# 23skdu/longbow

Measured on AMD Instinct MI355X. Metric: k-NN queries/sec (batch=1024, k=100), 1Mx768 f32, higher is better.
Workload: dtype f32

## Files before the change

### longbow_amd/csrc/kernels_gemm.hip

```cpp
#include "lb_admit.h"

#include <cstdlib>

namespace lb {

constexpr int BM = 128;
constexpr int BN = 128;
constexpr int BK = 32;
constexpr int GEMM_THREADS = 256;

struct GemmArgs {
    const float *X;
    const float *norm2;
    const float *rnorm;
    int64_t row_begin, row_end;
    int D;
    const float *Q;
    int nq;
    const uint8_t *mask;
    const uint32_t *rowmap;
    CandState cs;
    int n_row_tiles, n_q_tiles;
    int boot;
};

__device__ __forceinline__ int swz_off(int row, int chunk)
{
    return row * BK + ((chunk ^ ((row >> 1) & 7)) << 2);
}

template <int MODE>
__device__ __forceinline__ f32x4 load_chunk(const float *base, int64_t row, int D, int k)
{
    f32x4 v = {0.f, 0.f, 0.f, 0.f};
    const float *p = base + row * (int64_t)D + k;
    if (MODE == 2) {
        v = *reinterpret_cast<const f32x4 *>(p);
    } else if (MODE == 1) {
        if (k < D) v = *reinterpret_cast<const f32x4 *>(p);
    } else {
        if (k + 0 < D) v.x = p[0];
        if (k + 1 < D) v.y = p[1];
        if (k + 2 < D) v.z = p[2];
        if (k + 3 < D) v.w = p[3];
    }
    return v;
}

template <int METRIC, int ALIGNED>
__global__ __launch_bounds__(GEMM_THREADS, 2) void gemm_filter_kernel(GemmArgs a)
{
    constexpr bool GLDS = ALIGNED == 2;
    const int b = blockIdx.x;
    const int xcd = b & 7;
    const int in_xcd = b >> 3;
    const int qt = in_xcd % a.n_q_tiles;
    const int rt = (in_xcd / a.n_q_tiles) * 8 + xcd;
    if (rt >= a.n_row_tiles) return;

    __shared__ __attribute__((aligned(16))) float lds_all[2 * 2 * BM * BK + BM + BM + BM / 4];
    float(*lds)[2][BM * BK] = reinterpret_cast<float(*)[2][BM * BK]>(lds_all);
    float *s_aux = lds_all + 2 * 2 * BM * BK;
    uint32_t *s_rowid = reinterpret_cast<uint32_t *>(s_aux + BM);
    uint8_t *s_vis = reinterpret_cast<uint8_t *>(s_rowid + BM);

    const int tid = threadIdx.x;
    const int lane = tid & 63;
    const int wave = tid >> 6;
    const int wr = wave >> 1, wc = wave & 1;
    const int l31 = lane & 31, h = lane >> 5;

    const int64_t row0 = a.row_begin + (int64_t)rt * BM;
    const int q0 = qt * BN;
    const int64_t last_row = a.row_end - 1;
    const int last_q = a.nq - 1;

    auto corpus_row = [&](int64_t pos) -> int64_t {
        if (pos > last_row) pos = last_row;
        return a.rowmap ? (int64_t)a.rowmap[pos] : pos;
    };
    const int64_t side_ri = corpus_row(row0 + (tid & (BM - 1)));

    int st_row[4], st_ch[4];
    int64_t st_xrow[4];
    int st_qrow[4];
#pragma unroll
    for (int i = 0; i < 4; i++) {
        int c = tid + GEMM_THREADS * i;
        st_row[i] = c >> 3;
        st_ch[i] = c & 7;
        st_xrow[i] = corpus_row(row0 + st_row[i]);
        int qr = q0 + st_row[i];
        st_qrow[i] = qr < last_q ? qr : last_q;
    }

    f32x16 acc[2][2];
#pragma unroll
    for (int i = 0; i < 2; i++)
#pragma unroll
        for (int j = 0; j < 2; j++)
#pragma unroll
            for (int r = 0; r < 16; r++) acc[i][j][r] = 0.f;

    const int nk = (a.D + BK - 1) / BK;
    f32x4 ra[4], rb[4];

    const float *gsrcA[4], *gsrcB[4];
    if (GLDS) {
#pragma unroll
        for (int i = 0; i < 4; i++) {
            const int j = wave * 4 + i;
            const int row = j * 8 + (lane >> 3);
            const int c = (lane & 7) ^ ((row >> 1) & 7);
            const int64_t xr = corpus_row(row0 + row);
            int qr = q0 + row;
            if (qr > last_q) qr = last_q;
            gsrcA[i] = a.X + xr * (int64_t)a.D + 4 * c;
            gsrcB[i] = a.Q + (int64_t)qr * a.D + 4 * c;
        }
    }
    const int wave_u = __builtin_amdgcn_readfirstlane(wave);
    auto glds_piece = [&](int p, int stage, int k0) {
        const int i = p >> 1;
        const int j = wave_u * 4 + i;
        if ((p & 1) == 0)
            __builtin_amdgcn_global_load_lds(
                (const __attribute__((address_space(1))) void *)(gsrcA[i] + k0),
                (__attribute__((address_space(3))) void *)(&lds[stage][0][j * 8 * BK]), 16, 0,
                2);
        else
            __builtin_amdgcn_global_load_lds(
                (const __attribute__((address_space(1))) void *)(gsrcB[i] + k0),
                (__attribute__((address_space(3))) void *)(&lds[stage][1][j * 8 * BK]), 16, 0, 0);
    };
    auto glds_stage = [&](int stage, int k0) {
#pragma unroll
        for (int p = 0; p < 8; p++) glds_piece(p, stage, k0);
    };
    if (GLDS) glds_stage(0, 0);
    const float aux_r = side_aux<METRIC>(a.norm2, a.rnorm, side_ri);
    uint8_t side_vis = 1;
    if (a.mask) side_vis = a.mask[side_ri];
    uint64_t tau_raw[2];
#pragma unroll
    for (int tn = 0; tn < 2; tn++) {
        const int qj = q0 + wc * 64 + tn * 32 + l31;
        tau_raw[tn] = lane_tau(a.cs.tau, qj, a.nq, a.boot);
    }
    if (tid < BM) {
        s_aux[tid] = aux_r;
        s_vis[tid] = (row0 + tid <= last_row && side_vis) ? (uint8_t)1 : (uint8_t)0;
        s_rowid[tid] = (uint32_t)side_ri;
    }
    float tau_key[2];
    uint32_t tau_row[2];
#pragma unroll
    for (int tn = 0; tn < 2; tn++) {
        tau_key[tn] = tau_key_of(tau_raw[tn]);
        tau_row[tn] = entry_row(tau_raw[tn]);
    }
    if (!GLDS) {
#pragma unroll
        for (int i = 0; i < 4; i++) {
            ra[i] = load_chunk<ALIGNED>(a.X, st_xrow[i], a.D, st_ch[i] * 4);
            rb[i] = load_chunk<ALIGNED>(a.Q, st_qrow[i], a.D, st_ch[i] * 4);
        }
#pragma unroll
        for (int i = 0; i < 4; i++) {
            *reinterpret_cast<f32x4 *>(&lds[0][0][swz_off(st_row[i], st_ch[i])]) = ra[i];
            *reinterpret_cast<f32x4 *>(&lds[0][1][swz_off(st_row[i], st_ch[i])]) = rb[i];
        }
    }
    __syncthreads();

    if constexpr (GLDS) {
        struct Frag {
            f32x4 a[2], b[2];
        };
        auto ldfrag = [&](Frag &f, int stage, int s) {
            const float *As = lds[stage][0];
            const float *Bs = lds[stage][1];
            const int ch = 2 * s + h;
#pragma unroll
            for (int t = 0; t < 2; t++) {
                f.a[t] = *reinterpret_cast<const f32x4 *>(&As[swz_off(wr * 64 + t * 32 + l31, ch)]);
                f.b[t] = *reinterpret_cast<const f32x4 *>(&Bs[swz_off(wc * 64 + t * 32 + l31, ch)]);
            }
        };
        auto mfma16 = [&](const Frag &f) {
#pragma unroll
            for (int e = 0; e < 4; e++)
#pragma unroll
                for (int tm = 0; tm < 2; tm++)
#pragma unroll
                    for (int tn = 0; tn < 2; tn++)
                        acc[tm][tn] = __builtin_amdgcn_mfma_f32_32x32x2f32(f.a[tm][e], f.b[tn][e], acc[tm][tn], 0, 0, 0);
        };
        Frag F0, F1;
        auto steps012 = [&](int cur) {
            ldfrag(F1, cur, 1);
            mfma16(F0);
            ldfrag(F0, cur, 2);
            mfma16(F1);
            ldfrag(F1, cur, 3);
            mfma16(F0);
#pragma unroll
            for (int s = 0; s < 3; s++) {
                __builtin_amdgcn_sched_group_barrier(0x008, 2, 0);
                __builtin_amdgcn_sched_group_barrier(0x100, 4, 0);
                __builtin_amdgcn_sched_group_barrier(0x008, 14, 0);
            }
            __builtin_amdgcn_sched_barrier(0);
        };
        ldfrag(F0, 0, 0);
        if (nk > 1) glds_stage(1, BK);
        int kt = 0;
        for (; kt + 2 < nk; kt++) {
            const int cur = kt & 1;
            steps012(cur);
            __syncthreads();
            const int k0 = (kt + 2) * BK;
            ldfrag(F0, cur ^ 1, 0);
#pragma unroll
            for (int p = 0; p < 8; p++) glds_piece(p, cur, k0);
            mfma16(F1);
            __builtin_amdgcn_sched_group_barrier(0x008, 2, 0);
            __builtin_amdgcn_sched_group_barrier(0x100, 4, 0);
#pragma unroll
            for (int p = 0; p < 7; p++) {
                __builtin_amdgcn_sched_group_barrier(0x020, 1, 0);
                __builtin_amdgcn_sched_group_barrier(0x008, 2, 0);
            }
            __builtin_amdgcn_sched_group_barrier(0x020, 1, 0);
        }
        if (kt + 1 < nk) {
            const int cur = kt & 1;
            steps012(cur);
            __syncthreads();
            ldfrag(F0, cur ^ 1, 0);
            mfma16(F1);
            __builtin_amdgcn_sched_group_barrier(0x008, 2, 0);
            __builtin_amdgcn_sched_group_barrier(0x100, 4, 0);
            __builtin_amdgcn_sched_group_barrier(0x008, 14, 0);
            kt++;
        }
        steps012(kt & 1);
        mfma16(F1);
    } else {
        for (int kt = 0; kt < nk; kt++) {
            const int cur = kt & 1;
            const bool has_next = kt + 1 < nk;
            if (has_next) {
                const int k0 = (kt + 1) * BK;
#pragma unroll
                for (int i = 0; i < 4; i++) {
                    ra[i] = load_chunk<ALIGNED>(a.X, st_xrow[i], a.D, k0 + st_ch[i] * 4);
                    rb[i] = load_chunk<ALIGNED>(a.Q, st_qrow[i], a.D, k0 + st_ch[i] * 4);
                }
            }
            const float *As = lds[cur][0];
            const float *Bs = lds[cur][1];
            f32x4 fa[2][2], fb[2][2];
#pragma unroll
            for (int t = 0; t < 2; t++) {
                fa[0][t] = *reinterpret_cast<const f32x4 *>(&As[swz_off(wr * 64 + t * 32 + l31, h)]);
                fb[0][t] = *reinterpret_cast<const f32x4 *>(&Bs[swz_off(wc * 64 + t * 32 + l31, h)]);
            }
#pragma unroll
            for (int s = 0; s < 4; s++) {
                const int cb = s & 1, nb = cb ^ 1;
                if (s < 3) {
                    const int ch = 2 * (s + 1) + h;
#pragma unroll
                    for (int t = 0; t < 2; t++) {
                        fa[nb][t] = *reinterpret_cast<const f32x4 *>(&As[swz_off(wr * 64 + t * 32 + l31, ch)]);
                        fb[nb][t] = *reinterpret_cast<const f32x4 *>(&Bs[swz_off(wc * 64 + t * 32 + l31, ch)]);
                    }
                }
#pragma unroll
                for (int e = 0; e < 4; e++)
#pragma unroll
                    for (int tm = 0; tm < 2; tm++)
#pragma unroll
                        for (int tn = 0; tn < 2; tn++)
                            acc[tm][tn] = __builtin_amdgcn_mfma_f32_32x32x2f32(fa[cb][tm][e], fb[cb][tn][e],
                                                                              acc[tm][tn], 0, 0, 0);
                if (s == 1 && has_next) {
                    const int nxt = cur ^ 1;
#pragma unroll
                    for (int i = 0; i < 4; i++) {
                        *reinterpret_cast<f32x4 *>(&lds[nxt][0][swz_off(st_row[i], st_ch[i])]) = ra[i];
                        *reinterpret_cast<f32x4 *>(&lds[nxt][1][swz_off(st_row[i], st_ch[i])]) = rb[i];
                    }
                }
            }
            __syncthreads();
        }
    }

    float aux[2][4][4];
    uint32_t rid[2][4][4];
    uint32_t vbits = 0;
#pragma unroll
    for (int tm = 0; tm < 2; tm++)
#pragma unroll
        for (int g = 0; g < 4; g++)
            vbits |= tile_rows4(s_aux, s_rowid, s_vis, wr * 64 + tm * 32 + 8 * g + 4 * h, aux[tm][g], rid[tm][g]) << (tm * 16 + g * 4);
#pragma unroll
    for (int tn = 0; tn < 2; tn++) {
        const int qj = q0 + wc * 64 + tn * 32 + l31;
        const bool qok = qj < a.nq;
        uint64_t *list = a.cs.lists + (size_t)(qok ? qj : 0) * a.cs.cap;
        if (a.boot) {
            if (qok) {
#pragma unroll
                for (int tm = 0; tm < 2; tm++)
#pragma unroll
                    for (int g = 0; g < 4; g++) {
                        const int64_t rbase = row0 + wr * 64 + tm * 32 + 8 * g + 4 * h;
                        uint64_t ent[4];
#pragma unroll
                        for (int e = 0; e < 4; e++)
                            ent[e] = ((vbits >> (tm * 16 + g * 4 + e)) & 1u) ? pack_entry(cand_key<METRIC>(acc[tm][tn][4 * g + e], aux[tm][g][e]), rid[tm][g][e]) : kEntryMax;
                        uint64_t *dst = list + (rbase - a.row_begin);
                        if (rbase + 3 < a.row_end) {
                            typedef unsigned long long u64x2 __attribute__((ext_vector_type(2)));
                            u64x2 v0 = {ent[0], ent[1]}, v1 = {ent[2], ent[3]};
                            *reinterpret_cast<u64x2 *>(dst) = v0;
                            *reinterpret_cast<u64x2 *>(dst + 2) = v1;
                        } else {
#pragma unroll
                            for (int e = 0; e < 4; e++)
                                if (rbase + e < a.row_end) dst[e] = ent[e];
                        }
                    }
            }
            continue;
        }
        uint32_t bits = 0;
#pragma unroll
        for (int tm = 0; tm < 2; tm++)
#pragma unroll
            for (int g = 0; g < 4; g++)
#pragma unroll
                for (int e = 0; e < 4; e++)
                    bits |= admit_exact(cand_key<METRIC>(acc[tm][tn][4 * g + e], aux[tm][g][e]), rid[tm][g][e], tau_key[tn], tau_row[tn]) << (tm * 16 + g * 4 + e);
        bits &= vbits;
        if (bits) {
            uint32_t pos = atomicAdd(&a.cs.cnt[qj], (uint32_t)__builtin_popcount(bits));
#pragma unroll
            for (int tm = 0; tm < 2; tm++)
#pragma unroll
                for (int g = 0; g < 4; g++)
#pragma unroll
                    for (int e = 0; e < 4; e++)
                        if (bits & (1u << (tm * 16 + g * 4 + e))) {
                            const uint32_t ri = rid[tm][g][e];
                            if (pos < a.cs.cap) list[pos] = pack_entry(cand_key<METRIC>(acc[tm][tn][4 * g + e], aux[tm][g][e]), ri);
                            pos++;
                        }
        }
    }
}

__global__ __launch_bounds__(256) void split_bf16_kernel(const float *src, float *dst, int64_t n8)
{
    for (int64_t i = (int64_t)blockIdx.x * blockDim.x + threadIdx.x; i < n8; i += (int64_t)gridDim.x * blockDim.x) {
        bf16x8 hi, lo;
        split_bf16x8(*reinterpret_cast<const f32x4 *>(src + i * 8), *reinterpret_cast<const f32x4 *>(src + i * 8 + 4), hi, lo);
        const int64_t grp = i >> 1;
        const int kb = (int)(i & 1);
        char *g = reinterpret_cast<char *>(dst) + grp * 64;
        *reinterpret_cast<bf16x8 *>(g + kb * 16) = hi;
        *reinterpret_cast<bf16x8 *>(g + 32 + kb * 16) = lo;
    }
}

void launch_split_bf16(const float *src, float *dst, int64_t rows, int D, hipStream_t s)
{
    const int64_t n8 = rows * (int64_t)D / 8;
    if (n8 <= 0) return;
    int64_t blocks = (n8 + 255) / 256;
    if (blocks > 16384) blocks = 16384;
    hipLaunchKernelGGL(split_bf16_kernel, dim3((unsigned)blocks), dim3(256), 0, s, src, dst, n8);
}

void launch_gemm_filter(int metric, const float *X, const float *norm2, const float *rnorm,
                        int64_t row_begin, int64_t row_end, int D, const float *Q, int nq,
                        const uint8_t *mask, const uint32_t *rowmap, CandState cs, bool boot, hipStream_t s)
{
    if (row_end <= row_begin || nq <= 0) return;
    GemmArgs a;
    a.rowmap = rowmap;
    a.boot = boot ? 1 : 0;
    a.X = X; a.norm2 = norm2; a.rnorm = rnorm;
    a.row_begin = row_begin; a.row_end = row_end; a.D = D;
    a.Q = Q; a.nq = nq; a.mask = mask; a.cs = cs;
    a.n_row_tiles = (int)((row_end - row_begin + BM - 1) / BM);
    a.n_q_tiles = (nq + BN - 1) / BN;
    const int groups = (a.n_row_tiles + 7) / 8;
    dim3 grid((unsigned)(groups * 8 * a.n_q_tiles));
    const bool aligned = (D % 4 == 0) && ((reinterpret_cast<uintptr_t>(X) & 15) == 0) &&
                         ((reinterpret_cast<uintptr_t>(Q) & 15) == 0);
    const int mode = !aligned ? 0 : (D % BK == 0 ? 2 : 1);
#define LB_GEMM(M, AL) hipLaunchKernelGGL((gemm_filter_kernel<M, AL>), grid, dim3(GEMM_THREADS), 0, s, a)
#define LB_GEMM_M(M)                 \
    do {                             \
        if (mode == 2) LB_GEMM(M, 2); \
        else if (mode == 1) LB_GEMM(M, 1); \
        else LB_GEMM(M, 0);           \
    } while (0)
    if (metric == METRIC_L2) LB_GEMM_M(METRIC_L2);
    else if (metric == METRIC_COS) LB_GEMM_M(METRIC_COS);
    else LB_GEMM_M(METRIC_DOT);
#undef LB_GEMM_M
#undef LB_GEMM
}

}
```

Measured before the change: 86930.

## Stage admitted candidates in LDS list and flush per-query with block-level atomics

Admitted candidates from the GEMM filter are now appended to a shared-memory local list with per-query counters instead of each lane doing a global atomicAdd on the per-query count and scattering entries to global memory. At the end of the block a flush routine writes the collected entries to the global candidate lists, presumably reserving global space once per query per block. The boot path is hoisted out and returns early. This adds LDS usage (about 3K floats plus per-query counters), which may reduce occupancy, and falls back to direct global writes when the local list overflows.

```diff
diff --git a/longbow_amd/csrc/kernels_gemm.hip b/longbow_amd/csrc/kernels_gemm.hip
--- a/longbow_amd/csrc/kernels_gemm.hip
+++ b/longbow_amd/csrc/kernels_gemm.hip
@@ -58,11 +58,14 @@
     const int rt = (in_xcd / a.n_q_tiles) * 8 + xcd;
     if (rt >= a.n_row_tiles) return;
 
-    __shared__ __attribute__((aligned(16))) float lds_all[2 * 2 * BM * BK + BM + BM + BM / 4];
+    constexpr int FL_CAP = 1024;
+    constexpr int SIDE_F = BM + BM + BM / 4;
+    __shared__ __attribute__((aligned(16))) float lds_all[2 * 2 * BM * BK + SIDE_F + 3 * FL_CAP + 1 + 2 * BN];
     float(*lds)[2][BM * BK] = reinterpret_cast<float(*)[2][BM * BK]>(lds_all);
     float *s_aux = lds_all + 2 * 2 * BM * BK;
     uint32_t *s_rowid = reinterpret_cast<uint32_t *>(s_aux + BM);
     uint8_t *s_vis = reinterpret_cast<uint8_t *>(s_rowid + BM);
+    const LocalList<FL_CAP, BN, GEMM_THREADS> fl(reinterpret_cast<uint32_t *>(s_aux + SIDE_F + 3 * FL_CAP), reinterpret_cast<uint64_t *>(s_aux + SIDE_F));
 
     const int tid = threadIdx.x;
     const int lane = tid & 63;
@@ -152,6 +155,7 @@
         s_vis[tid] = (row0 + tid <= last_row && side_vis) ? (uint8_t)1 : (uint8_t)0;
         s_rowid[tid] = (uint32_t)side_ri;
     }
+    fl.reset(tid);
     float tau_key[2];
     uint32_t tau_row[2];
 #pragma unroll
@@ -306,61 +310,87 @@
 #pragma unroll
         for (int g = 0; g < 4; g++)
             vbits |= tile_rows4(s_aux, s_rowid, s_vis, wr * 64 + tm * 32 + 8 * g + 4 * h, aux[tm][g], rid[tm][g]) << (tm * 16 + g * 4);
+    if (a.boot) {
+#pragma unroll
+        for (int tn = 0; tn < 2; tn++) {
+            const int qj = q0 + wc * 64 + tn * 32 + l31;
+            if (qj >= a.nq) continue;
+            uint64_t *list = a.cs.lists + (size_t)qj * a.cs.cap;
+#pragma unroll
+            for (int tm = 0; tm < 2; tm++)
+#pragma unroll
+                for (int g = 0; g < 4; g++) {
+                    const int64_t rbase = row0 + wr * 64 + tm * 32 + 8 * g + 4 * h;
+                    uint64_t ent[4];
+#pragma unroll
+                    for (int e = 0; e < 4; e++)
+                        ent[e] = ((vbits >> (tm * 16 + g * 4 + e)) & 1u) ? pack_entry(cand_key<METRIC>(acc[tm][tn][4 * g + e], aux[tm][g][e]), rid[tm][g][e]) : kEntryMax;
+                    uint64_t *dst = list + (rbase - a.row_begin);
+                    if (rbase + 3 < a.row_end) {
+                        typedef unsigned long long u64x2 __attribute__((ext_vector_type(2)));
+                        u64x2 v0 = {ent[0], ent[1]}, v1 = {ent[2], ent[3]};
+                        *reinterpret_cast<u64x2 *>(dst) = v0;
+                        *reinterpret_cast<u64x2 *>(dst + 2) = v1;
+                    } else {
+#pragma unroll
+                        for (int e = 0; e < 4; e++)
+                            if (rbase + e < a.row_end) dst[e] = ent[e];
+                    }
+                }
+        }
+        return;
+    }
+    uint32_t bits[2];
 #pragma unroll
     for (int tn = 0; tn < 2; tn++) {
-        const int qj = q0 + wc * 64 + tn * 32 + l31;
-        const bool qok = qj < a.nq;
-        uint64_t *list = a.cs.lists + (size_t)(qok ? qj : 0) * a.cs.cap;
-        if (a.boot) {
-            if (qok) {
-#pragma unroll
-                for (int tm = 0; tm < 2; tm++)
-#pragma unroll
-                    for (int g = 0; g < 4; g++) {
-                        const int64_t rbase = row0 + wr * 64 + tm * 32 + 8 * g + 4 * h;
-                        uint64_t ent[4];
-#pragma unroll
-                        for (int e = 0; e < 4; e++)
-                            ent[e] = ((vbits >> (tm * 16 + g * 4 + e)) & 1u) ? pack_entry(cand_key<METRIC>(acc[tm][tn][4 * g + e], aux[tm][g][e]), rid[tm][g][e]) : kEntryMax;
-                        uint64_t *dst = list + (rbase - a.row_begin);
-                        if (rbase + 3 < a.row_end) {
-                            typedef unsigned long long u64x2 __attribute__((ext_vector_type(2)));
-                            u64x2 v0 = {ent[0], ent[1]}, v1 = {ent[2], ent[3]};
-                            *reinterpret_cast<u64x2 *>(dst) = v0;
-                            *reinterpret_cast<u64x2 *>(dst + 2) = v1;
-                        } else {
-#pragma unroll
-                            for (int e = 0; e < 4; e++)
-                                if (rbase + e < a.row_end) dst[e] = ent[e];
+        bits[tn] = 0;
+#pragma unroll
+        for (int tm = 0; tm < 2; tm++)
+#pragma unroll
+            for (int g = 0; g < 4; g++)
+#pragma unroll
+                for (int e = 0; e < 4; e++)
+                    bits[tn] |= admit_exact(cand_key<METRIC>(acc[tm][tn][4 * g + e], aux[tm][g][e]), rid[tm][g][e], tau_key[tn], tau_row[tn]) << (tm * 16 + g * 4 + e);
+        bits[tn] &= vbits;
+    }
+#pragma unroll
+    for (int tn = 0; tn < 2; tn++) {
+        if (!bits[tn]) continue;
+        const int ql = wc * 64 + tn * 32 + l31;
+        const uint32_t n = (uint32_t)__builtin_popcount(bits[tn]);
+        uint32_t lp = atomicAdd(fl.cnt, n);
+        if (lp + n <= (uint32_t)fl.CAP) {
+            uint32_t lr = atomicAdd(&fl.qcnt[ql], n);
+#pragma unroll
+            for (int tm = 0; tm < 2; tm++)
+#pragma unroll
+                for (int g = 0; g < 4; g++)
+#pragma unroll
+                    for (int e = 0; e < 4; e++)
+                        if (bits[tn] & (1u << (tm * 16 + g * 4 + e))) {
+                            fl.ent[lp] = pack_entry(cand_key<METRIC>(acc[tm][tn][4 * g + e], aux[tm][g][e]), rid[tm][g][e]);
+                            fl.q[lp] = (uint16_t)ql;
+                            fl.rk[lp] = (uint16_t)lr;
+                            lp++;
+                            lr++;
                         }
-                    }
-            }
-            continue;
-        }
-        uint32_t bits = 0;
-#pragma unroll
-        for (int tm = 0; tm < 2; tm++)
-#pragma unroll
-            for (int g = 0; g < 4; g++)
-#pragma unroll
-                for (int e = 0; e < 4; e++)
-                    bits |= admit_exact(cand_key<METRIC>(acc[tm][tn][4 * g + e], aux[tm][g][e]), rid[tm][g][e], tau_key[tn], tau_row[tn]) << (tm * 16 + g * 4 + e);
-        bits &= vbits;
-        if (bits) {
-            uint32_t pos = atomicAdd(&a.cs.cnt[qj], (uint32_t)__builtin_popcount(bits));
+        } else {
+            fl.reserved_unused(lp, n);
+            uint64_t *list = a.cs.lists + (size_t)(q0 + ql) * a.cs.cap;
+            uint32_t pos = atomicAdd(&a.cs.cnt[q0 + ql], n);
 #pragma unroll
             for (int tm = 0; tm < 2; tm++)
 #pragma unroll
                 for (int g = 0; g < 4; g++)
 #pragma unroll
                     for (int e = 0; e < 4; e++)
-                        if (bits & (1u << (tm * 16 + g * 4 + e))) {
-                            const uint32_t ri = rid[tm][g][e];
-                            if (pos < a.cs.cap) list[pos] = pack_entry(cand_key<METRIC>(acc[tm][tn][4 * g + e], aux[tm][g][e]), ri);
+                        if (bits[tn] & (1u << (tm * 16 + g * 4 + e))) {
+                            if (pos < a.cs.cap) list[pos] = pack_entry(cand_key<METRIC>(acc[tm][tn][4 * g + e], aux[tm][g][e]), rid[tm][g][e]);
                             pos++;
                         }
         }
     }
+    fl.flush(tid, a.cs, q0);
 }
 
 __global__ __launch_bounds__(256) void split_bf16_kernel(const float *src, float *dst, int64_t n8)
```

New measurement: 86870, median of 2. No clear change (-0.1%).
